# Nat-zewge/cuda-PHDSLAM

Hardware: AMD Instinct MI355X
Metric: PHD update steps/sec at N_particles x N_gm x N_meas; achieved HBM GB/s vs roofline (higher is better)
Workload: dtype f32

## Files before the change

### cuda-phdslam_amd/csrc/phd_kernels.h

```cpp
#pragma once
#include <hip/hip_runtime.h>

#include <cstddef>
#include <cstdint>

#include "phd_device.h"
#include "phd_types.h"

#define PHD_ZBINS 256
#define PHD_STAMP_SLOTS 52
#define UPD_THREADS_MIN 256
#define UPD_THREADS_MAX 1024
#define PHD_CPHD_MAX_M 127
#if defined(PHD_EXPERIMENT) && PHD_EXPERIMENT == 4
#define PHD_CPHD_SEG 2
#elif defined(PHD_EXPERIMENT) && PHD_EXPERIMENT == 5
#define PHD_CPHD_SEG 1
#else
#define PHD_CPHD_SEG 4
#endif

#define PHD_ST_SURVIVOR_OVERFLOW 1
#define PHD_ST_CANDIDATE_OVERFLOW 2
#define PHD_ST_MAP_OVERFLOW 4
#define PHD_ST_SERIAL_MERGE 8
#define PHD_ST_ETA_RANGE 16
#define PHD_ST_PAIR_OVERFLOW 32
#define PHD_ST_WAIT_TIMEOUT 64
#define PHD_ST_INFO (PHD_ST_SERIAL_MERGE | PHD_ST_PAIR_OVERFLOW)

#include <string>

namespace phd {

struct PredictCfg {
    int index_offset;
    float dt;
    int subdivide;
    float l, h, a, b;
    float stdAlpha, stdEncoder;
    float ax, ay, ayaw;
};

struct RsStepArgs {
    const float* w;
    float* w_out;
    int N, B, has_meas;
    float resample_thresh, new_logw;
    uint64_t seed, step;
    double* part_s2;
    unsigned long long *cdf_rel, *part_tot, *part_key;
    unsigned* sync;
    float* out;
    int* parents;
    const phd_pose* pose;
    const int* src;
    phd_pose* new_pose;
    int* new_src;
    float* logw;
    int* err;
};

#define RS_LEAD_WGS 8

struct UpdateArgs {
    int n, cap, M, Mcap, Kcap, Scap;
    int Epool;
    int plreq;
    int Bbuckets;
    int merge_mode;
    const int* slots;
    int first;
    int prio;
    int order;
    unsigned char* hand;
    const int* src;
    int* src_reset;
    const float* map_x;
    const int* size_x;
    const float* map_in;
    float* map_out;
    const int* size_in;
    int* size_out;
    phd_pose* poses;
    float* logw;
    float* logw_out;
    float* delta;
    const float* zr;
    const float* zb;
    const int* zok;
    const float4* zs;
    const unsigned short* zbin;
    int Mv;
    int zwide;
    int* status;
    int* err;
    unsigned long long* stamps;
    int predict;
    phd_ackerman_control pu;
    PredictCfg pc;
    uint64_t pseed, pstep;
    const phd_pose* pose_prior;
    const float* logw_prior;
    float* births;
    int Mb;
    const float* bzr;
    const float* bzb;
    const int* bzvi;
    double* cn_coef;
    int cn_stride;
    const double* lfact;
    int Nmax;
    DevCfg c;
    int rs_lead;
    RsStepArgs rs;
};

__host__ __device__ inline int upd_particle(const UpdateArgs& a, int b, int grid) {
    if (a.slots) return a.slots[b];
    const int g8 = grid & ~7;
    if (a.order == 1 && b < g8) b = g8 - 8 - (b & ~7) + (b & 7);
    return a.first + b;
}

struct UpdLds {
    size_t zr, zb, zok, leta, zs, etafx, etalo, zbin, out, cnt, scr, red, redf, pose, uni, thr;
    size_t u;
    size_t detv;
    size_t mpar, moff, mcur, medge, mpool;
    size_t in, near, skey, skey2;
    size_t skeyidx, gstart;
    size_t total;
    int B;
};

__host__ __device__ inline size_t upd_align16(size_t x) { return (x + 15) & ~(size_t)15; }

#ifndef PHD_RS_OVERLAP
#define PHD_RS_OVERLAP 3
#endif
#ifndef PHD_RS_LEAD
#define PHD_RS_LEAD 1
#endif


#ifndef PHD_PARTC_BMAX
#define PHD_PARTC_BMAX 1024
#endif
static_assert(PHD_PARTC_BMAX == 1024 || PHD_PARTC_BMAX == 2048 || PHD_PARTC_BMAX == 4096,
              "PHD_PARTC_BMAX: 1024, 2048 or 4096 buckets");

__host__ __device__ inline int upd_buckets(int Kcap, int part = 0) {
    return Kcap <= 768 && part == 2 ? 512 : Kcap <= 1024 ? 1024 : Kcap <= 2048 ? 2048 : Kcap <= 8192 ? 4096 : 16384;
}

__host__ __device__ inline int upd_epool(int Kcap) { return (3 * Kcap) / 2 + 16; }

__host__ __device__ inline UpdLds upd_lds_layout(int cap, int Mcap, int Kcap, int Scap, int Epool, int NT,
                                                  int cphd = 0, int part = 0) {
    UpdLds L;
    const int B = upd_buckets(Kcap, part);
    size_t o = 0;
    const bool pz = part != 0;
    L.zr = o;
    o = upd_align16(o + (pz ? 0 : 4 * (size_t)Mcap));
    L.zb = o;
    o = upd_align16(o + (pz ? 0 : 4 * (size_t)Mcap));
    L.zok = o;
    o = upd_align16(o + (pz ? 0 : 4 * (size_t)Mcap));
    L.leta = o;
    o = upd_align16(o + (pz && !(part == 2 && !cphd) ? 0 : 4 * (size_t)Mcap));
    const bool pc = part == 2;
    const bool pa = part == 1;
    L.zs = o;
    o = upd_align16(o + (pc ? 0 : 16 * (size_t)Mcap));
    L.etafx = o;
    o = upd_align16(o + (pc ? 0 : 8 * (size_t)Mcap));
    L.etalo = o;
    o = upd_align16(o + (pc ? 0 : 8 * (size_t)Mcap));
    L.zbin = o;
    o = upd_align16(o + (pc ? 0 : 2 * (size_t)PHD_ZBINS));
    L.out = o;
    o = upd_align16(o + (pc || pa ? 0 : 2 * (size_t)cap));
    L.cnt = o;
    o = upd_align16(o + 4 * 16);
    L.scr = o;
    o = upd_align16(o + (pc ? 4 * 2 * (size_t)(NT / 64) : 4 * 64));
    L.red = o;
    o = upd_align16(o + (pc ? 8 * 4 * (size_t)(NT / 64) : 8 * 64));
    L.redf = o;
    o = upd_align16(o + (pc ? 4 * (32 + (size_t)(NT / 64)) : 4 * 64));
    L.pose = o;
    o = upd_align16(o + sizeof(phd_pose));
    L.uni = o;
    o = upd_align16(o + 8 * 8);
    L.thr = o;
    o = upd_align16(o + (cphd && !pz ? 4 * (size_t)Mcap : 0));
    const size_t c0 = o;
    L.u = o;
    size_t m = c0 + 16 * (size_t)Kcap;
    L.detv = m;
    m = upd_align16(m + (pc ? 0 : 16 * ((size_t)Scap + (cphd ? 0 : (size_t)Mcap))));
    L.mcur = m;
    m = upd_align16(m + 2 * ((size_t)Kcap + 2));
    L.medge = m;
    m = upd_align16(m + 4 * (size_t)Epool);
    L.mpar = m;
    m = upd_align16(m + 2 * (size_t)Kcap);
    L.moff = L.mcur;
    L.mpool = m;
    m = upd_align16(m + 4 * (size_t)Epool);
    size_t table = c0 + (size_t)cap * (8 * 4) + 16 + 2 * (size_t)NT;
    o = upd_align16(part == 1 || (part != 2 && table > m) ? table : m);
    const size_t d0 = o;
    L.in = o;
    o = upd_align16(o + (pc || pa ? 0 : 2 * (size_t)cap));
    L.near = o;
    o = upd_align16(o + (pc || pa ? 0 : 2 * (size_t)cap));
    const size_t skb = upd_align16(4 * ((size_t)Scap + 4));
    if (pc && L.mpool + 4 * (size_t)Epool >= L.mcur + 2 * skb) {
        L.skey = L.mcur;
        L.skey2 = L.mcur + skb;
    } else {
        L.skey = o;
        o = upd_align16(o + (pa ? 0 : skb));
        L.skey2 = o;
        o = upd_align16(o + (pa ? 0 : skb));
    }
    const size_t d_a = o;
    o = d0;
    L.skeyidx = o;
    o = upd_align16(o + 2 * (size_t)Kcap);
    L.B = B;
    int Bp = 0;
    if (part == 2) {
        const int bmin = B > 1024 ? B : 1024;
        for (int b = PHD_PARTC_BMAX > bmin ? PHD_PARTC_BMAX : bmin; b >= bmin && !Bp; b >>= 1)
            if (L.mpar - L.mcur >= 2 * ((size_t)b + 2)) Bp = b;
    }
    if (Bp) {
        L.B = Bp;
        L.gstart = L.mcur;
    } else {
        L.gstart = o;
        o = upd_align16(o + 2 * ((size_t)L.B + 2));
    }
    L.total = (part == 1 || o <= d_a) ? d_a : o;
    return L;
}

struct CphdHand {
    size_t cnt, sums, ehi, elo, in, near, out, skey, leta, thr, misc, detv, table, rb, stride;
};
#define HAND_GIN 0
#define HAND_GNEAR 1
#define HAND_GOUT 2
#define HAND_NSURV 3
#define HAND_FLAGS 4
__host__ __device__ inline CphdHand cphd_hand_layout(int cap, int Mcap, int Scap) {
    CphdHand H;
    size_t o = 0;
    H.cnt = o;
    o += 64;
    H.sums = o;
    o += 32;
    H.ehi = o;
    o = upd_align16(o + 8 * (size_t)Mcap);
    H.elo = o;
    o = upd_align16(o + 8 * (size_t)Mcap);
    H.in = o;
    o = upd_align16(o + 2 * (size_t)cap);
    H.near = o;
    o = upd_align16(o + 2 * (size_t)cap);
    H.out = o;
    o = upd_align16(o + 2 * (size_t)cap);
    H.skey = o;
    o = upd_align16(o + 4 * (size_t)Scap);
    H.leta = o;
    o = upd_align16(o + 4 * (size_t)Mcap);
    H.thr = o;
    o = upd_align16(o + 4 * (size_t)Mcap);
    H.misc = o;
    o = upd_align16(o + 16);
    H.detv = o;
    o = upd_align16(o + 16 * ((size_t)Scap + (size_t)Mcap));
    H.table = o;
    o = upd_align16(o + 32 * (size_t)cap + 16 + 2 * 1024);
    H.rb = o;
    o = upd_align16(o + 8 * (size_t)cap);
    H.stride = (o + 255) & ~(size_t)255;
    return H;
}

__global__ void k_predict_ackerman(phd_pose* poses, int n, phd_ackerman_control u, const phd_ackerman_noise* noise_in,
                                   PredictCfg c, uint64_t seed, uint64_t step, const phd_pose* pose_prior,
                                   const float* logw_prior, float* logw, const int* slots);
__global__ void k_expand(int n, int npp, const phd_pose* pose, const int* src, const float* logw, phd_pose* new_pose,
                         int* new_src, float* new_logw, float log_npp);
__global__ void k_predict_cv(phd_pose* poses, int n, const phd_cv_noise* noise_in, PredictCfg c, uint64_t seed,
                             uint64_t step, const phd_pose* pose_prior, const float* logw_prior, float* logw,
                             const int* slots);
__global__ void k_update_fused_256(UpdateArgs a);
__global__ void k_update_fused_512(UpdateArgs a);
__global__ void k_update_fused_1024(UpdateArgs a);
__global__ void k_update_cphd_a_256(UpdateArgs a);
__global__ void k_update_cphd_a_512(UpdateArgs a);
__global__ void k_update_cphd_a_1024(UpdateArgs a);
__global__ void k_update_cphd_a_p256(UpdateArgs a);
__global__ void k_update_cphd_a_p512(UpdateArgs a);
__global__ void k_update_cphd_c_256(UpdateArgs a);
__global__ void k_update_cphd_c_512(UpdateArgs a);
__global__ void k_update_cphd_c_1024(UpdateArgs a);
__global__ void k_update_phd_a_256(UpdateArgs a);
__global__ void k_update_phd_a_512(UpdateArgs a);
__global__ void k_update_phd_a_1024(UpdateArgs a);
__global__ void k_update_phd_c_256(UpdateArgs a);
__global__ void k_update_phd_c_512(UpdateArgs a);
__global__ void k_update_phd_c_1024(UpdateArgs a);
__global__ void k_cphd_terms(UpdateArgs a);
inline size_t cphd_terms_lds(int Mcap) { return (size_t)7 * 8 * ((size_t)Mcap + 4); }
__global__ void k_cphd_cardinality(const int* src, const double* cn_coef, const double* cn_x, int stride,
                                   const double* lfact, int Nmax, int n, float* out);
__global__ void k_update_fused_p256(UpdateArgs a);
__global__ void k_update_fused_p512(UpdateArgs a);
__global__ void k_update_fused_256_h(UpdateArgs a);
__global__ void k_update_fused_512_h(UpdateArgs a);
__global__ void k_update_fused_1024_h(UpdateArgs a);
__global__ void k_update_fused_p256_h(UpdateArgs a);
__global__ void k_update_fused_p512_h(UpdateArgs a);
__global__ void k_update_phd_c_256_h(UpdateArgs a);
__global__ void k_update_phd_c_512_h(UpdateArgs a);
__global__ void k_update_phd_c_1024_h(UpdateArgs a);
__global__ void k_update_cphd_c_256_h(UpdateArgs a);
__global__ void k_update_cphd_c_512_h(UpdateArgs a);
__global__ void k_update_cphd_c_1024_h(UpdateArgs a);
__global__ void k_normalize(float* logw, int n, const float* lse_override, float* out, float resample_thresh,
                            int has_meas);
__global__ void k_lse_parts(const float* logw, int n, float* out);
__global__ void k_resample(const int* flag, const float* logw_in, float* logw_out, int n, int n_out,
                           const double* u_in,
                           uint64_t seed, uint64_t step, unsigned long long* cdf, int* idx, phd_pose* pose, int* src,
                           phd_pose* tmp_pose, int* tmp_src, float new_logw);
#define RS_LDS_MAX 8192
__global__ void k_normalize_resample(float* logw, int n, float* out, float resample_thresh, int has_meas, uint64_t seed,
                                     uint64_t step, unsigned long long* cdf, int* idx, phd_pose* pose, int* src,
                                     phd_pose* tmp_pose, int* tmp_src, float new_logw);
__global__ void k_apply_parents(const int* flag, const int* idx, int n, phd_pose* pose, int* src, float* logw,
                                phd_pose* tmp_pose, int* tmp_src, float new_logw);
__global__ void k_add_births(int* src, const int* slots, int n, int cap, const float* map_in, const int* size_in,
                             const float* map_x, const int* size_x, float* map_out, int* size_out,
                             const phd_pose* pose, const float* zr, const float* zb, const int* zok, int M, DevCfg c,
                             int* status, int* err);
#define RS_THREADS 1024
#define RS_STAGE_CHUNKS 4
#define RS_MAX_CHUNKS 1024
__global__ void k_rs_max(const float* w, int N, float* part_max);
__global__ void k_rs_sum(const float* w, int N, const float* part_max, int B, double* part_sum, int max_of_w);
__global__ void k_rs_cdf(float* w, int N, const float* part_max, const double* part_sum, int B, double* part_s2,
                         unsigned long long* cdf_rel, unsigned long long* part_tot, unsigned long long* part_key,
                         float* out);
__global__ void k_rs_search(int N, int B, const double* part_s2, const unsigned long long* part_tot,
                            const unsigned long long* part_key, const unsigned long long* cdf_rel,
                            float resample_thresh, int has_meas, uint64_t seed, uint64_t step, int* parents,
                            float* out, const phd_pose* pose, const int* src, phd_pose* new_pose, int* new_src,
                            float* logw, float new_logw, const float* w_norm, unsigned* beyond);
__global__ void k_rs_sumcdf(const float* w, float* w_out, int N, int B, double* part_s2, unsigned long long* cdf_rel,
                            unsigned long long* part_tot, unsigned long long* part_key, float* out);
#define MIG_SENT 0
#define MIG_LSE 1
#define MIG_NEFF 2
#define MIG_FLAG 3
#define MIG_PENDING 4
#define MIG_OVF_SEND 5
#define MIG_OVF_RECV 6
#define MIG_OVF_CAP 7
#define MIG_TIMEOUT 8
#define MIG_SEQ 9
#define MIG_TAIL 10
#define PLAN_ARRIVE0 0
#define PLAN_ARRIVE1 1
// ... 63 lines not shown
```

### cuda-phdslam_amd/csrc/phd_kernels.hip

```cpp
#include <hip/hip_runtime.h>

#include <climits>
#include <cstdint>

#include "phd_detmath.h"
#include "phd_device.h"
#include "phd_kernels.h"
#include "phd_rng.h"
#include "phd_devutil.h"
#include "phd_cphd_terms.h"
#include "phd_block.h"
#include "phd_slab.h"

#ifdef PHD_STAMPS
#define STAMP(k)                                                                                  \
    do {                                                                                          \
        if (threadIdx.x == 0 && a.stamps) a.stamps[(size_t)blockIdx.x * PHD_STAMP_SLOTS + (k)] = __builtin_amdgcn_s_memtime(); \
    } while (0)
#else
#define STAMP(k) \
    do {         \
    } while (0)
#endif
#ifdef PHD_PLAN_STAMPS
// ... 1016 lines not shown
            {
                const int j0 = next_member(-1);
                if (j0 == i && next_member(i) == INT_MAX) {
                    emit_single(dst, cap, slot, X.K.P[i], X.K.V(i));
                    continue;
                }
            }
            for (int j = next_member(-1); j != INT_MAX; j = next_member(j)) {
                const float4 pj = X.K.P[j];
                W += (double)pj.z;
                sx += (double)(pj.z * pj.x);
                sy += (double)(pj.z * pj.y);
            }
            Wf = (float)W;
            const float rW = 1.0f / Wf;
            gx = (float)sx * rW;
            gy = (float)sy * rW;
            for (int j = next_member(-1); j != INT_MAX; j = next_member(j)) {
                const float4 pj = X.K.P[j], vj = X.K.V(j);
                const float d0 = gx - pj.x, d1 = gy - pj.y, w = pj.z;
                cv[0] += (double)(w * (vj.x + d0 * d0));
                cv[1] += (double)(w * (vj.y + d0 * d1));
                cv[2] += (double)(w * (vj.z + d1 * d0));
                cv[3] += (double)(w * (vj.w + d1 * d1));
            }
        }
        emit_merged(dst, cap, slot, Wf, gx, gy, cv);
    }
    return nout;
}

template <bool PRED>
__device__ __forceinline__ phd_pose fused_predict(const UpdateArgs& a, int n) {
    phd_pose ps = a.pose_prior ? a.pose_prior[n] : a.poses[n];
    if (a.logw_prior) a.logw[n] = a.logw_prior[n];
    if (PRED && a.predict) {
        for (int k = 0; k < a.pc.subdivide; k++) {
            const uint64_t st = a.pstep * (uint64_t)a.pc.subdivide + (uint64_t)k;
            if (a.predict == 1) {
                float n_alpha, n_enc;
                ackerman_noise(a.pseed, a.pc.index_offset + n, st, a.pc, &n_alpha, &n_enc);
                ps = predict_ackerman_one(ps, a.pu, n_alpha, n_enc, a.pc);
            } else {
                ps = predict_cv_one(ps, cv_noise(a.pseed, a.pc.index_offset + n, st, a.pc), a.pc);
            }
        }
        a.poses[n] = ps;
    }
    return ps;
}

__global__ void __launch_bounds__(256)
    k_cphd_cardinality(const int* __restrict__ src, const double* __restrict__ cn_coef,
                       const double* __restrict__ cn_x, int stride, const double* __restrict__ lfact, int Nmax,
                       int n, float* __restrict__ out) {
    const int p = blockIdx.x;
    if (p >= n) return;
    const double* co = slab_cn(src ? src[p] : p, cn_coef, cn_x, stride);
    const double ip0 = co[0], lq = co[1], lw = co[2], logW = co[3], W = co[4];
    const int M = (int)co[5];
    for (int k = threadIdx.x; k <= Nmax; k += blockDim.x) {
        double mx = -INFINITY;
        if (k > 0 && !(W > 0)) {
            out[(size_t)p * (Nmax + 1) + k] = PHD_LOG0;
            continue;
        }
        for (int j = 0; j <= min(k, M); j++) {
            const double b = co[6 + j];
            if (b == -INFINITY) continue;
            const double t = b + (k > 0 ? (double)k * logW : 0.0) - W - lfact[k - j] +
                             (k - j > 0 ? (double)(k - j) * lq : 0.0) - (k > 0 ? (double)k * lw : 0.0);
            mx = fmax(mx, t);
        }
        double sum = 0.0;
        if (mx != -INFINITY)
            for (int j = 0; j <= min(k, M); j++) {
                const double b = co[6 + j];
                if (b == -INFINITY) continue;
                const double t = b + (k > 0 ? (double)k * logW : 0.0) - W - lfact[k - j] +
                                 (k - j > 0 ? (double)(k - j) * lq : 0.0) - (k > 0 ? (double)k * lw : 0.0);
                sum += exp(t - mx);
            }
        out[(size_t)p * (Nmax + 1) + k] = mx == -INFINITY ? PHD_LOG0 : (float)(log(sum) + mx - ip0);
    }
}

__device__ __forceinline__ unsigned int bearing_window(float C2, float S0, float S12, float S3, float bearing,
                                                       float floor2, int Mv, const unsigned short* s_zbin) {
    const float k2 = 0.72134752044448170f;
    unsigned int win = (unsigned int)Mv << 16;
    if (!(C2 > floor2) && C2 == C2) return 0;
    const float kap = S3 - S12 * S12 * __builtin_amdgcn_rcpf(4.f * S0);
    if (S0 > 0.f && kap > 0.f && kap < INFINITY && C2 < 1e30f) {
        const float hw = sqrtf(2.f * (C2 - floor2) * __builtin_amdgcn_rcpf(k2 * kap)) * 1.001f + 1e-4f;
        const float ibinw = PHD_ZBINS / 6.28318530717958648f;
        const int ba = (int)floorf((bearing - hw + 3.14159265358979f) * ibinw) - 1;
        const int bc = (int)floorf((bearing + hw + 3.14159265358979f) * ibinw) + 2;
        if (bc - ba < PHD_ZBINS) {
            const int fa = ba >= 0 ? ba / PHD_ZBINS : -((PHD_ZBINS - 1 - ba) / PHD_ZBINS);
            const int fc = bc >= 0 ? bc / PHD_ZBINS : -((PHD_ZBINS - 1 - bc) / PHD_ZBINS);
            const int ia = s_zbin[ba - fa * PHD_ZBINS] + fa * Mv;
            const int ic = s_zbin[bc - fc * PHD_ZBINS] + fc * Mv;
            const int lo = ia - fa * Mv;
            win = (unsigned int)lo | ((unsigned int)min(ic - ia, Mv) << 16);
        }
    }
    return win;
}

__device__ __forceinline__ void eta_term(unsigned long long* ehi, unsigned long long* elo, int m, float q,
                                         float lo_scale, int& flags) {
    flags |= q >= 1048576.f ? PHD_ST_ETA_RANGE : 0;
    const bool hi = q >= 7.62939453125e-06f;
    const unsigned long long y = (unsigned long long)(fminf(q, 4194304.f) * (hi ? 1099511627776.f : lo_scale));
#if PHD_XK == 11
    if (y) (hi ? ehi : elo)[m] += y;
#else
    if (y) atomicAdd((hi ? ehi : elo) + m, y);
#endif
}

template <int NT>
__device__ void rs_step_block(const RsStepArgs& a, unsigned char* smem);

template <int NT, bool PRED, bool CPHD = false, int PART = 0, int METRIC = 0>
__device__ __forceinline__ void update_body(const UpdateArgs& a) {
    static_assert(!CPHD || PART != 0, "the CPHD update runs as three launches (part A, k_cphd_terms, part C)");
    extern __shared__ __attribute__((aligned(16))) unsigned char smem[];
    const int lead = PART == 2 ? a.rs_lead : 0;
    if (PART == 2 && (int)blockIdx.x < lead) {
        if (blockIdx.x == 0) rs_step_block<NT>(a.rs, smem);
        return;
    }
    const int b_ = (int)blockIdx.x - lead, grid_ = (int)gridDim.x - lead;
    const UpdLds L = upd_lds_layout(a.cap, a.Mcap, a.Kcap, a.Scap, a.Epool, NT, CPHD ? 1 : 0, PART);
    float* s_zr = (float*)(smem + L.zr);
    float* s_zb = (float*)(smem + L.zb);
    int* s_zok = (int*)(smem + L.zok);
    float* s_leta = (float*)(smem + L.leta);
    float* s_thr = (float*)(smem + L.thr);
    const float4* s_zs = PART == 2 ? a.zs : (const float4*)(smem + L.zs);
    unsigned long long* s_etafx = (unsigned long long*)(smem + L.etafx);
    unsigned long long* s_etalo = (unsigned long long*)(smem + L.etalo);
    const unsigned short* s_zbin = PART == 2 ? a.zbin : (const unsigned short*)(smem + L.zbin);
    unsigned short* s_out = (unsigned short*)(smem + L.out);
    int* s_cnt = (int*)(smem + L.cnt);
    int* s_scr = (int*)(smem + L.scr);
    double* s_red = (double*)(smem + L.red);
    float* s_redf = (float*)(smem + L.redf);
    unsigned short* s_in = (unsigned short*)(smem + L.in);
    unsigned short* s_near = (unsigned short*)(smem + L.near);
    unsigned int* s_skey = (unsigned int*)(smem + L.skey);
    unsigned int* s_skey2 = (unsigned int*)(smem + L.skey2);
    float4* t_a = (float4*)(smem + L.u);
    float2* t_b = (float2*)(smem + L.u + 16 * (size_t)a.cap);
    unsigned int* t_w = (unsigned int*)(smem + L.u + 24 * (size_t)a.cap);
    int* t_pre = (int*)(smem + L.u + 28 * (size_t)a.cap);
    unsigned short* t_start = (unsigned short*)(smem + L.u + 32 * (size_t)a.cap + 16);
    MergeScratch X;
    X.K.P = (float4*)(smem + L.u);
    X.K.detv = (float4*)(smem + L.detv);
    X.K.cap = a.cap;
    X.par = (short*)(smem + L.mpar);
    X.off = (unsigned short*)(smem + L.moff);
    X.cur = (unsigned short*)(smem + L.mcur);
    X.edges = (unsigned int*)(smem + L.medge);
    X.pool = (unsigned short*)(smem + L.mpool);
    X.plist = (unsigned int*)(smem + L.mpar);
    X.plcap = (int)((L.mpool + 4 * (size_t)a.Epool - L.mpar) / 4);
    X.key = (unsigned short*)(smem + L.skeyidx);
    X.gstart = (unsigned short*)(smem + L.gstart);
    X.st_tests = nullptr;

    const int n = upd_particle(a, b_, grid_);
    const int tid = threadIdx.x;
#ifdef PHD_STAMPS
    if (tid == 0 && a.stamps) a.stamps[(size_t)blockIdx.x * PHD_STAMP_SLOTS + 48] = __builtin_amdgcn_s_memrealtime();
#endif
    const DevCfg& c = a.c;
    const int M = a.M;
    const int sref = a.src ? a.src[n] : n;
    const bool in_x = (sref & PHD_SLAB_X) != 0;
    const int slab = sref & PHD_SLAB_MASK;
    const int G = in_x ? a.size_x[slab] : a.size_in[slab];
    const G1 float* __restrict__ src = g1(uni_p((in_x ? a.map_x : a.map_in) + (size_t)slab * PHD_NF * a.cap));
    const int Mb = a.births ? max(0, min(a.Mb, a.cap - G)) : 0;
    const int Gp = G + Mb;
    G1 float* __restrict__ bdst = a.births ? g1(uni_p(a.births + (size_t)n * PHD_NF * a.cap)) : nullptr;
    const G1 float* __restrict__ bsrc = a.births ? bdst - G : src;
    auto prior = [&](int k) -> const G1 float* { return (k < G ? src : bsrc) + k; };
    X.K.src = src;
    X.K.bsrc = bsrc;
    X.K.G = G;
    G1 float* __restrict__ dst = g1(uni_p(a.map_out + (size_t)n * PHD_NF * a.cap));
    phd_pose& s_pose = *(phd_pose*)(smem + L.pose);
    double* s_uni = (double*)(smem + L.uni);
    if (b_ >= grid_ - a.prio) __builtin_amdgcn_s_setprio(3);
    const CphdHand H = cphd_hand_layout(a.cap, a.Mcap, a.Scap);
    unsigned char* hand = PART ? a.hand + (size_t)n * H.stride : nullptr;
    if (PART == 1) {
        s_out = (unsigned short*)(hand + H.out);
        s_in = (unsigned short*)(hand + H.in);
        s_near = (unsigned short*)(hand + H.near);
        s_skey = (unsigned int*)(hand + H.skey);
    }
    if (PART == 2) {
        s_out = (unsigned short*)(hand + H.out);
        s_in = (unsigned short*)(hand + H.in);
        s_near = (unsigned short*)(hand + H.near);
        X.K.detv = (float4*)(hand + H.detv);
        s_zr = const_cast<float*>(a.zr);
        s_zb = const_cast<float*>(a.zb);
        s_zok = const_cast<int*>(a.zok);
        if (CPHD) {
            s_leta = (float*)(hand + H.leta);
            s_thr = (float*)(hand + H.thr);
        }
        unsigned char* tb = hand + H.table;
        t_a = (float4*)tb;
        t_b = (float2*)(tb + 16 * (size_t)a.cap);
        t_w = (unsigned int*)(tb + 24 * (size_t)a.cap);
        t_pre = (int*)(tb + 28 * (size_t)a.cap);
        t_start = (unsigned short*)(tb + 32 * (size_t)a.cap + 16);
    }
    constexpr int PF = 2;
    float pf[PF][PHD_NF];
#pragma unroll
    for (int it = 0; it < PF; it++) {
        const int k = it * NT + tid;
#pragma unroll
        for (int f = 0; f < PHD_NF; f++) pf[it][f] = (k < G) ? src[f * a.cap + k] : 0.f;
    }
    int hp_cnt[5] = {0, 0, 0, 0, 0};
    unsigned int hp_skey = 0;
    float hp_leta = 0.f, hp_thr = 0.f, hp_nd = 0.f;
    int hp_wide = 0;
    unsigned long long hp_eta[2] = {0ull, 0ull};
    if constexpr (PART == 2) {
        const int* hc = (const int*)(hand + H.cnt);
#pragma unroll
        for (int i = 0; i < 5; i++) hp_cnt[i] = hc[i];
        if (tid < a.Scap) hp_skey = ((const unsigned int*)(hand + H.skey))[tid];
        if (CPHD) {
            if (tid < M) {
                hp_leta = ((const float*)(hand + H.leta))[tid];
                hp_thr = ((const float*)(hand + H.thr))[tid];
            }
            hp_nd = ((const float*)(hand + H.misc))[0];
            hp_wide = ((const int*)(hand + H.misc))[1];
        } else if (tid < M) {
            hp_eta[0] = ((const unsigned long long*)(hand + H.ehi))[tid];
            hp_eta[1] = ((const unsigned long long*)(hand + H.elo))[tid];
        }
    }
    if (tid == 0) s_pose = fused_predict<PRED && PART != 2>(a, n);

    const int Mv = a.Mv;
    for (int m = tid; m < M; m += NT) {
        if (PART == 0) {
            s_zr[m] = a.zr[m];
            s_zb[m] = a.zb[m];
            s_zok[m] = a.zok[m];
        }
        if (PART != 2) {
            s_etafx[m] = 0ull;
            s_etalo[m] = 0ull;
        }
    }
    if (PART != 2) {
        for (int m = tid; m < Mv; m += NT) ((float4*)(smem + L.zs))[m] = a.zs[m];
        for (int b = tid; b < PHD_ZBINS; b += NT) ((unsigned short*)(smem + L.zbin))[b] = a.zbin[b];
    }
    if (tid < 16) s_cnt[tid] = 0;
    __syncthreads();
    const phd_pose pose = s_pose;
    STAMP(0);

    const float k2 = 0.72134752044448170f;
    double card_d = 0.0;
    double win_d = 0.0, qd_d = 0.0, wall_d = 0.0;
    int n1r = 0, n2r = 0, n0r = 0;
    constexpr int NW = NT / 64;
    const float lpd = d_safe_log(c.pd);
    for (int base = 0; base < (PART == 2 ? 0 : Gp); base += NT) {
        const int k = base + tid;
        int cls = -1;
        float4 ta = make_float4(0.f, 0.f, 0.f, 0.f);
        float2 tb = make_float2(0.f, 0.f);
        unsigned int win = 0;
        if (k < Gp) {
            float v[PHD_NF];
            if (k >= G) {
                const int m = a.bzvi[k - G];
                float mean[2], cov[4];
                d_birth(c, pose.px, pose.py, pose.ptheta, a.bzr[m], a.bzb[m], mean, cov);
                v[0] = c.birthWeight;
                v[1] = mean[0];
                v[2] = mean[1];
                v[3] = cov[0];
                v[4] = cov[1];
                v[5] = cov[2];
                v[6] = cov[3];
#pragma unroll
                for (int f = 0; f < PHD_NF; f++) bdst[f * a.cap + (k - G)] = v[f];
            } else if (base == 0) {
#pragma unroll
                for (int f = 0; f < PHD_NF; f++) v[f] = pf[0][f];
            } else if (base == NT) {
#pragma unroll
                for (int f = 0; f < PHD_NF; f++) v[f] = pf[1][f];
            } else {
#pragma unroll
                for (int f = 0; f < PHD_NF; f++) v[f] = src[f * a.cap + k];
            }
            const float dx = v[1] - pose.px;
            const float dy = v[2] - pose.py;
            const float r2 = dx * dx + dy * dy;
            const float r = sqrtf(r2);
            const float bearing = d_wrap((PHD_XK == 13 ? atan2f(dy, dx) : phd_atan2f(dy, dx)) - pose.ptheta);
            const float ab = fabsf(bearing);
            if (CPHD) wall_d += (double)v[0];
            if (r >= c.minRange && r <= c.maxRange && ab <= c.maxBearing)
                cls = 1;
            else if ((double)r >= 0.8 * (double)c.minRange && (double)r <= 1.2 * (double)c.maxRange &&
                     (double)ab <= 1.2 * (double)c.maxBearing)
                cls = 2;
            else
                cls = 0;
            if (cls == 1) {
                const float w = v[0];
                DevEkf e;
                d_ekf_from_geometry(c, dx, dy, r2, r, bearing, v[3], v[4], v[5], v[6], e);
                const double lc =
                    (double)((e.pd > 0.f ? lpd : PHD_LOG0) + d_safe_log(w)) - c.log_2pi - 0.5 * (double)d_safe_log(e.det);
                const float C2 = (float)(1.4426950408889634 * lc);
                const float S12 = e.S1 + e.S2;
                ta = make_float4(e.r, e.bearing, e.S0, S12);
                tb = make_float2(e.S3, C2);
                card_d += (double)(e.pd * w);
                if (CPHD) {
                    win_d += (double)w;
                    qd_d += (double)(1 - e.pd) * (double)w;
                }
                win = bearing_window(C2, e.S0, S12, e.S3, e.bearing, c.walk_floor, Mv, s_zbin);
            }
        }
        const int lane = tid & 63, wid = tid >> 6;
        const unsigned long long b1 = __ballot(cls == 1), b2 = __ballot(cls == 2), b0 = __ballot(cls == 0);
        const unsigned long long lt = (1ull << lane) - 1ull;
        int* sb = s_scr + 16 + ((base / NT) & 1) * 3 * NW;
        if (lane == 0) {
            sb[wid] = __popcll(b1);
            sb[NW + wid] = __popcll(b2);
            sb[2 * NW + wid] = __popcll(b0);
        }
        __syncthreads();
        int o1 = n1r, o2 = n2r, o0 = n0r, t1 = 0, t2 = 0, t0 = 0;
#pragma unroll
        for (int w = 0; w < NW; w++) {
            const int c1 = sb[w], c2 = sb[NW + w], c0 = sb[2 * NW + w];
            if (w < wid) {
                o1 += c1;
                o2 += c2;
                o0 += c0;
            }
            t1 += c1;
            t2 += c2;
            t0 += c0;
        }
        if (cls == 1) {
            const int j = o1 + __popcll(b1 & lt);
            s_in[j] = (unsigned short)k;
            t_a[j] = ta;
            t_b[j] = tb;
            t_w[j] = win;
            if (PART == 1) {
                G1 float* rbp = (G1 float*)(hand + H.rb) + 2 * j;
                rbp[0] = ta.x;
                rbp[1] = ta.y;
            }
        }
        if (cls == 2) s_near[o2 + __popcll(b2 & lt)] = (unsigned short)k;
        if (cls == 0) s_out[o0 + __popcll(b0 & lt)] = (unsigned short)k;
        n1r += t1;
        n2r += t2;
        n0r += t0;
    }
    if (PART != 2 && tid == 0) {
        s_cnt[0] = n1r;
        s_cnt[1] = n2r;
        s_cnt[2] = n0r;
    }
    int Gin = PART == 2 ? s_cnt[0] : n1r;
    STAMP(1);
    if constexpr (PART == 2) {
    } else if (CPHD) {
        double v[4] = {card_d, win_d, qd_d, wall_d};
        block_sum<4, NT>(v, s_red);
        if (tid == 0) {
            s_uni[0] = v[0];
            s_uni[1] = v[1];
            s_uni[2] = v[2];
            s_uni[3] = v[3];
        }
    } else {
        double v[1] = {card_d};
        block_sum<1, NT>(v, s_red);
        if (tid == 0) s_uni[0] = v[0];
    }
    STAMP(2);
    {
        const float thr2 = c.lq_keep_thresh * 1.4426950408889634f;
        const float lo_scale = a.cap <= 2047 ? 1.1805916207174113e21f : 1.152921504606846976e18f;
        const int lane = tid & 63;
        const unsigned long long lt = (1ull << lane) - 1ull;
        int eflags = 0;
        int W = 0, chunk = 0;
        auto plan_walk = [&]() {
            W = 0;
            for (int base = 0; base < Gin; base += NT) {
                const int j = base + tid;
                const int units = j < Gin ? (int)((t_w[j] >> 16) + 3) >> 2 : 0;
                int tot;
                const int pre = block_excl_scan<NT>(units, s_scr, &tot);
                if (j < Gin) t_pre[j] = W + pre;
                W += tot;
// ... 8 lines not shown
            __syncthreads();
        };
        auto walk = [&](const int pass) {
        const bool do_sum = pass == 0;
        const float thr_u = CPHD ? c.cphd_thr0 : thr2;
        const int w0 = tid * chunk, w1 = min(w0 + chunk, W);
#ifdef PHD_STAMPS
        int st_pairs = 0, st_qpos = 0;
#endif
        int j = w0 < w1 ? t_start[tid] : 0;
        STAMP(25);
        int jbeg = t_pre[j], jend = t_pre[j + 1];
        for (int it = 0; it < (PHD_XK == 1 ? 0 : chunk); it++) {
            const int w = w0 + it;
            const bool act = w < w1;
            if (act && w == jend) {
                j++;
                while (t_pre[j + 1] <= w) j++;
                jbeg = t_pre[j];
                jend = t_pre[j + 1];
            }
            const float4 ta = t_a[j];
            const float2 tb = t_b[j];
            const unsigned int win = t_w[j];
            const int cnt = act ? (int)(win >> 16) : 0;
            const int e0 = 4 * (w - jbeg);
            int ms = (int)(win & 0xffffu) + (act ? e0 : 0);
            while (ms >= Mv) ms -= Mv;
            float4 z[4];
#pragma unroll
            for (int k = 0; k < 4; k++) {
                z[k] = s_zs[ms];
                ms = (ms + 1 == Mv) ? 0 : ms + 1;
            }
            float l2q[4];
            int mm[4];
#pragma unroll
            for (int k = 0; k < 4; k++) {
                const float i0 = z[k].x - ta.x;
                float i1 = z[k].y - ta.y;
                if (fabsf(i1) > 3.14159250f) i1 = d_wrap(i1);
                const float u = __builtin_fmaf(i0, ta.z, i1 * ta.w);
                const float dist = __builtin_fmaf(i0, u, i1 * i1 * tb.x);
                l2q[k] = e0 + k < cnt ? __builtin_fmaf(-k2, dist, tb.y) : -INFINITY;
                mm[k] = __float_as_int(z[k].z);
            }
            if (do_sum) {
#pragma unroll
                for (int k = 0; k < 4; k++) {
                    const float q = __builtin_amdgcn_exp2f(l2q[k]);
                    if (PHD_XK != 12 && q > 0.f) eta_term(s_etafx, s_etalo, mm[k], q, lo_scale, eflags);
#ifdef PHD_STAMPS
                    st_pairs += e0 + k < cnt;
                    st_qpos += q > 0.f;
#endif
                }
            }
            bool lst[4];
#pragma unroll
            for (int k = 0; k < 4; k++) lst[k] = l2q[k] >= (pass == 0 ? thr_u : s_thr[e0 + k < cnt ? mm[k] : 0]);
            unsigned long long bl[4];
#pragma unroll
            for (int k = 0; k < 4; k++) bl[k] = __ballot(lst[k]);
            const int c0 = __popcll(bl[0]), c1 = __popcll(bl[1]), c2 = __popcll(bl[2]), c3 = __popcll(bl[3]);
            const int ntot = c0 + c1 + c2 + c3;
            if (ntot) {
                int base = 0;
                if (lane == 0) base = atomicAdd(&s_cnt[3], ntot);
                base = __shfl(base, 0, 64);
                const int off[4] = {base, base + c0, base + c0 + c1, base + c0 + c1 + c2};
#pragma unroll
                for (int k = 0; k < 4; k++) {
                    const int sl = off[k] + __popcll(bl[k] & lt);
                    if (lst[k] && sl < a.Scap) s_skey[sl] = ((unsigned int)mm[k] << 16) | (unsigned int)j;
                }
            }
        }
#ifdef PHD_STAMPS
        atomicAdd(&s_cnt[8 + pass], st_pairs);
        atomicAdd(&s_cnt[10 + pass], st_qpos);
#endif
        if (eflags) atomicOr(&s_cnt[14], eflags);
        __syncthreads();
        };
        if constexpr (PART != 2) {
        plan_walk();
#ifdef PHD_STAMPS
        if (tid == 0) s_cnt[12] = W;
#endif
        STAMP(21);
        walk(0);
        if constexpr (PART == 1) {
            int* hc = (int*)(hand + H.cnt);
            if (tid == 0) {
                hc[HAND_GIN] = Gin;
                hc[HAND_GNEAR] = s_cnt[1];
                hc[HAND_GOUT] = s_cnt[2];
                hc[HAND_NSURV] = s_cnt[3];
                hc[HAND_FLAGS] = s_cnt[14];
            }
            if (tid < 4) ((double*)(hand + H.sums))[tid] = s_uni[tid];
            for (int m = tid; m < M; m += NT) {
                ((unsigned long long*)(hand + H.ehi))[m] = s_etafx[m];
                ((unsigned long long*)(hand + H.elo))[m] = s_etalo[m];
            }
            if constexpr (!CPHD) {
                static_assert(NT >= 256, "one measurement per thread (M <= 256)");
                float lt = 0.f;
                if (tid < M) {
                    float sum;
                    if (Gin > 0) {
                        double sd = (double)s_etafx[tid] * 9.094947017729282e-13 +
                                    (double)s_etalo[tid] * (a.cap <= 2047 ? 8.470329472543003e-22 : 8.673617379884035e-19);
                        sd += (double)c.kappa;
                        sd += (double)c.birthWeight;
                        sum = (float)sd;
                    } else {
                        sum = c.kappa + c.birthWeight;
                    }
                    lt = d_det_safe_log(sum);
                }
                __syncthreads();
                if (tid < M) ((float*)s_etafx)[tid] = lt;
                __syncthreads();
                if (tid == 0) {
                    float pw = 0.f;
                    for (int m = 0; m < M; m++) pw += ((const float*)s_etafx)[m];
                    const float cardp = (float)(s_uni[0] + (double)M * (double)c.birthWeight);
                    const float delta = pw - cardp;
                    a.delta[n] = delta;
                    const float nw = a.logw[n] + delta;
                    a.logw[n] = nw;
                    if (a.logw_out) a.logw_out[n] = nw;
                }
            }
            STAMP(9);
            return;
        }
        } else {
            if (tid == 0) {
                s_cnt[0] = hp_cnt[HAND_GIN];
                s_cnt[1] = hp_cnt[HAND_GNEAR];
                s_cnt[2] = hp_cnt[HAND_GOUT];
                s_cnt[3] = hp_cnt[HAND_NSURV];
                s_cnt[14] = hp_cnt[HAND_FLAGS];
                ((float*)(s_uni + 4))[0] = hp_nd;
                ((float*)(s_uni + 4))[1] = phd_det_expf(hp_nd);
                s_uni[5] = (double)hp_wide;
                if (!CPHD) s_uni[0] = ((const double*)(hand + H.sums))[0];
            }
            Gin = hp_cnt[HAND_GIN];
            const int nsk = min(hp_cnt[HAND_NSURV], a.Scap);
            for (int q = tid; q < nsk; q += NT) s_skey[q] = q == tid ? hp_skey : ((const unsigned int*)(hand + H.skey))[q];
            __syncthreads();
            if (CPHD && (s_uni[5] != 0.0 || s_cnt[3] > a.Scap)) {
                float tm = INFINITY;
                for (int m = tid; m < M; m += NT) tm = fminf(tm, s_thr[m]);
                const float fl = fminf(c.walk_floor, -block_max_f<NT>(-tm, s_redf) - 1.f);
                for (int q = tid; q < Gin; q += NT) {
                    const int k = s_in[q];
                    const G1 float* sk = prior(k);
                    const float dx = sk[1 * a.cap] - pose.px;
                    const float dy = sk[2 * a.cap] - pose.py;
                    const float r2 = dx * dx + dy * dy;
                    const float r = sqrtf(r2);
                    const float bearing = d_wrap(phd_atan2f(dy, dx) - pose.ptheta);
                    DevEkf e;
                    d_ekf_from_geometry(c, dx, dy, r2, r, bearing, sk[3 * a.cap], sk[4 * a.cap], sk[5 * a.cap],
                                        sk[6 * a.cap], e);
                    const double lc = (double)(d_safe_log(e.pd) + d_safe_log(sk[0])) - c.log_2pi -
                                      0.5 * (double)d_safe_log(e.det);
                    const float C2 = (float)(1.4426950408889634 * lc);
                    const float S12 = e.S1 + e.S2;
                    t_a[q] = make_float4(e.r, e.bearing, e.S0, S12);
                    t_b[q] = make_float2(e.S3, C2);
                    t_w[q] = bearing_window(C2, e.S0, S12, e.S3, e.bearing, fl, Mv, s_zbin);
                }
                __syncthreads();
                plan_walk();
                if (tid == 0) s_cnt[3] = 0;
                __syncthreads();
                walk(1);
            }
        }
        STAMP(22);
        if (!CPHD && tid < M) {
            float sum;
            if (Gin > 0) {
                const unsigned long long ehi = PART == 2 ? hp_eta[0] : s_etafx[tid];
                const unsigned long long elo = PART == 2 ? hp_eta[1] : s_etalo[tid];
                double sd = (double)ehi * 9.094947017729282e-13 +
                            (double)elo * (a.cap <= 2047 ? 8.470329472543003e-22 : 8.673617379884035e-19);
                sd += (double)c.kappa;
                sd += (double)c.birthWeight;
                sum = (float)sd;
            } else {
                sum = c.kappa + c.birthWeight;
            }
            s_leta[tid] = d_det_safe_log(sum);
        }
        __syncthreads();
    }
    if (!CPHD && PART != 2 && tid == 0) {
        float pw = 0.f;
        for (int m = 0; m < M; m++) pw += s_leta[m];
        const float cardp = (float)(s_uni[0] + (double)M * (double)c.birthWeight);
        const float delta = pw - cardp;
        a.delta[n] = delta;
        const float nw = a.logw[n] + delta;
        a.logw[n] = nw;
        if (a.logw_out) a.logw_out[n] = nw;
    }
    STAMP(3);
    int nsurv = s_cnt[3];
    int flags = s_cnt[14];
    if (Mb < (a.births ? a.Mb : 0)) flags |= PHD_ST_MAP_OVERFLOW;
    if (nsurv > a.Scap) {
        flags |= PHD_ST_SURVIVOR_OVERFLOW;
        nsurv = a.Scap;
    }

    {
        int* b_cnt = (int*)(smem + L.u);
        int* b_base = b_cnt + 264;
        unsigned short* b_pos = (unsigned short*)(b_base + 264);
        unsigned int* b_tmp = (unsigned int*)(smem + L.u + 2 * 264 * 4 + upd_align16(2 * (size_t)a.Scap));
        for (int m = tid; m <= M; m += NT) b_cnt[m] = 0;
        __syncthreads();
        for (int s = tid; s < nsurv; s += NT)
            b_pos[s] = (unsigned short)atomicAdd(&b_cnt[s_skey[s] >> 16], 1);
        __syncthreads();
        {
            int run = 0;
            for (int base = 0; base < M; base += NT) {
                const int m = base + tid;
                int tot;
                const int pre = block_excl_scan<NT>(m < M ? b_cnt[m] : 0, s_scr, &tot);
                if (m < M) b_base[m] = run + pre;
                run += tot;
            }
        }
        __syncthreads();
        for (int s = tid; s < nsurv; s += NT) {
            const unsigned int key = s_skey[s];
            b_tmp[b_base[key >> 16] + b_pos[s]] = key;
        }
        __syncthreads();
        for (int s = tid; s < nsurv; s += NT) {
            const unsigned int key = s_skey[s];
            const int m = (int)(key >> 16), b0 = b_base[m], nb = b_cnt[m];
            int r = 0;
            for (int q = 0; q < nb; q++) r += b_tmp[b0 + q] < key;
            s_skey2[b0 + r] = key;
        }
        __syncthreads();
    }

    STAMP(4);
    int ncand = 0;
    int sbc = 0;
    int sc_bad = 0;
    float sc_lmax = 0.f;
    for (int base = 0; base < (PHD_XK == 4 ? 0 : Gin); base += NT) {
        const int j = base + tid;
        float w = 0.f;
        bool keep = false;
        int k = 0;
        float v[PHD_NF];
        if (j < Gin) {
            k = s_in[j];
            if (PART == 2 && base == 0 && k == j && k < G) {
#pragma unroll
                for (int f = 0; f < PHD_NF; f++) v[f] = pf[0][f];
            } else if (PART == 2 && base == NT && k == j && k < G) {
#pragma unroll
                for (int f = 0; f < PHD_NF; f++) v[f] = pf[1][f];
            } else {
#pragma unroll
                for (int f = 0; f < PHD_NF; f++) v[f] = prior(k)[f * a.cap];
            }
            w = CPHD ? (v[0] > 0.f ? v[0] * ((const float*)(s_uni + 4))[1] : 0.f) : v[0] * (1 - c.pd);
            keep = !(w < c.minFeatureWeight);
        }
        int tot;
        const int r = block_rank<NT, false>(keep, sb_at<NT>(s_scr, sbc), &tot);
        if (keep) {
            const int p = ncand + r;
            if (p < a.Kcap) {
                const float4 vc = make_float4(v[3], v[4], v[5], v[6]);
                X.K.P[p] = cand_record<METRIC>(v[1], v[2], w, vc, c.minSeparation, sc_bad, sc_lmax, (unsigned)k);
            }
        }
        ncand += tot;
    }
    STAMP(5);
    const int nd0 = min(ncand, a.Kcap);
    for (int base = 0; base < (PHD_XK == 4 ? 0 : nsurv); base += NT) {
        const int s = base + tid;
        bool keep = false;
        float w = 0.f, mx = 0.f, my = 0.f;
        DevEkf e;
        if (s < nsurv) {
            const unsigned int key = s_skey2[s];
            const int m = (int)(key >> 16);
            const int j = (int)(key & 0xffffu);
            const int k = s_in[j];
            const G1 float* sk = prior(k);
            mx = sk[1 * a.cap];
            my = sk[2 * a.cap];
            if constexpr (PART == 2) {
                const G1 float* rbp = (const G1 float*)(hand + H.rb) + 2 * j;
                const float dx = mx - s_pose.px, dy = my - s_pose.py;
                d_ekf_from_geometry(c, dx, dy, dx * dx + dy * dy, rbp[0], rbp[1], sk[3 * a.cap], sk[4 * a.cap],
                                    sk[5 * a.cap], sk[6 * a.cap], e);
            } else {
                d_compute_ekf(c, s_pose.px, s_pose.py, s_pose.ptheta, mx, my, sk[3 * a.cap], sk[4 * a.cap],
                              sk[5 * a.cap], sk[6 * a.cap], e);
            }
            const float i0 = s_zr[m] - e.r;
            const float i1 = d_wrap(s_zb[m] - e.bearing);
            const float dist = i0 * i0 * e.S0 + i0 * i1 * (e.S1 + e.S2) + i1 * i1 * e.S3;
            const float g = (float)(-0.5 * (double)dist - c.log_2pi - 0.5 * (double)d_safe_log(e.det));
            const float lq = d_safe_log(e.pd) + d_safe_log(sk[0]) + g;
            w = expf(lq - s_leta[m]);
            keep = !(w < c.minFeatureWeight);
            mx = mx + e.K0 * i0 + e.K2 * i1;
            my = my + e.K1 * i0 + e.K3 * i1;
        }
        int tot;
        const int r = block_rank<NT, false>(keep, sb_at<NT>(s_scr, sbc), &tot);
        if (keep) {
            const int p = ncand + r;
            if (p < a.Kcap) {
                const float4 v = make_float4(e.cu0, e.cu1, e.cu2, e.cu3);
                X.K.P[p] = cand_record<METRIC>(mx, my, w, v, c.minSeparation, sc_bad, sc_lmax,
                                               0x8000u | (unsigned)(p - nd0));
                X.K.detv[p - nd0] = v;
            }
        }
        ncand += tot;
    }
    STAMP(6);
    for (int base = 0; base < (CPHD ? 0 : M); base += NT) {
        const int m = base + tid;
        bool keep = false;
        float w = 0.f;
        if (m < M) {
            const float lb = s_zok[m] ? c.log_birth : PHD_LOG0;
            w = expf(lb - s_leta[m]);
            keep = !(w < c.minFeatureWeight);
        }
        int tot;
        const int r = block_rank<NT, false>(keep, sb_at<NT>(s_scr, sbc), &tot);
        if (keep) {
            const int p = ncand + r;
            if (p < a.Kcap) {
                float mean[2], cov[4];
                d_birth(c, s_pose.px, s_pose.py, s_pose.ptheta, s_zr[m], s_zb[m], mean, cov);
                const float4 v = make_float4(cov[0], cov[1], cov[2], cov[3]);
                X.K.P[p] = cand_record<METRIC>(mean[0], mean[1], w, v, c.minSeparation, sc_bad, sc_lmax,
                                               0x8000u | (unsigned)(p - nd0));
                X.K.detv[p - nd0] = v;
            }
        }
        ncand += tot;
    }
    const int Gnear = s_cnt[1];
    for (int q = tid; q < Gnear; q += NT) {
        const int p = ncand + q;
        if (p < a.Kcap) {
            const int k = s_near[q];
            const G1 float* sk = prior(k);
            const float4 v = make_float4(sk[3 * a.cap], sk[4 * a.cap], sk[5 * a.cap], sk[6 * a.cap]);
            X.K.P[p] = cand_record<METRIC>(sk[1 * a.cap], sk[2 * a.cap], sk[0], v, c.minSeparation, sc_bad, sc_lmax,
                                           (unsigned)k);
        }
    }
    ncand += Gnear;
    if (ncand > a.Kcap) {
        flags |= PHD_ST_CANDIDATE_OVERFLOW;
        ncand = a.Kcap;
    }
    __syncthreads();

    STAMP(7);
    int nout = (PHD_XK == 3 || PHD_XK == 4) ? 0
               : a.merge_mode != 0         ? -1
                                           : merge_parallel<NT, METRIC>(X, ncand, c.minSeparation, dst, a.cap, a.Epool,
                                                                        a.Bbuckets, s_scr, s_redf, s_cnt + 3, sc_bad,
                                                                        sc_lmax, a);
    if (nout < 0) {
        __syncthreads();
        nout = merge_serial<NT, METRIC>(X.K, nullptr, ncand, X.par, c.minSeparation, dst, a.cap, s_red, s_redf);
        flags |= PHD_ST_SERIAL_MERGE;
    }

    STAMP(8);
    flags |= s_cnt[14] & PHD_ST_PAIR_OVERFLOW;
    const int Gout = s_cnt[2];
    for (int q = tid; q < Gout; q += NT) {
        const int p = nout + q;
        if (p < a.cap) {
            const int k = s_out[q];
#pragma unroll
            for (int f = 0; f < PHD_NF; f++) st_out(dst + f * a.cap + p, prior(k)[f * a.cap]);
        }
    }
    int total = nout + Gout;
    if (total > a.cap) {
        flags |= PHD_ST_MAP_OVERFLOW;
        total = a.cap;
    }
    if (tid == 0) {
        a.size_out[n] = total;
        a.status[n] = flags;
        if (flags & ~PHD_ST_INFO) {
            atomicOr(a.err, flags & ~PHD_ST_INFO);
            atomicAdd(a.err + 3, 1);
        }
        if (flags & PHD_ST_SERIAL_MERGE) atomicAdd(a.err + 1, 1);
        if (a.src_reset) a.src_reset[n] = n;
    }
    STAMP(9);
#ifdef PHD_STAMPS
    if (tid == 0 && a.stamps) a.stamps[(size_t)blockIdx.x * PHD_STAMP_SLOTS + 49] = __builtin_amdgcn_s_memrealtime();
    if (tid == 0 && a.stamps) a.stamps[(size_t)blockIdx.x * PHD_STAMP_SLOTS + 10] = ((unsigned long long)ncand << 32) | (unsigned)nsurv;
    if (tid == 0 && a.stamps) {
        a.stamps[(size_t)blockIdx.x * PHD_STAMP_SLOTS + 40] = ((unsigned long long)s_cnt[8] << 32) | (unsigned)s_cnt[10];
        a.stamps[(size_t)blockIdx.x * PHD_STAMP_SLOTS + 41] = ((unsigned long long)s_cnt[9] << 32) | (unsigned)s_cnt[11];
        a.stamps[(size_t)blockIdx.x * PHD_STAMP_SLOTS + 42] = ((unsigned long long)Gin << 32) | (unsigned)s_cnt[12];
    }
#endif
}

typedef const __attribute__((address_space(4))) UpdateArgs KArgs;
__device__ __forceinline__ const UpdateArgs& kargs(const UpdateArgs& a) {
    (void)a;
    unsigned long long v = (unsigned long long)__builtin_amdgcn_kernarg_segment_ptr();
    asm volatile("" : "+s"(v));
    return *(const UpdateArgs*)(KArgs*)v;
}

__global__ void __launch_bounds__(256) k_update_fused_256(UpdateArgs a) { update_body<256, false>(kargs(a)); }
__global__ void __launch_bounds__(512) __attribute__((amdgpu_waves_per_eu(6, 8))) k_update_fused_512(UpdateArgs a) {
    update_body<512, false>(kargs(a));
}
__global__ void __launch_bounds__(1024) k_update_fused_1024(UpdateArgs a) { update_body<1024, false>(kargs(a)); }
__global__ void __launch_bounds__(256) k_update_fused_p256(UpdateArgs a) { update_body<256, true>(kargs(a)); }
#define PHD_CPHD_WPE __attribute__((amdgpu_waves_per_eu(4, 8)))
__global__ void __launch_bounds__(512) k_update_fused_p512(UpdateArgs a) { update_body<512, true>(kargs(a)); }
__global__ void __launch_bounds__(256) __attribute__((amdgpu_waves_per_eu(6, 8))) k_update_cphd_a_256(UpdateArgs a) {
    update_body<256, false, true, 1>(kargs(a));
}
__global__ void __launch_bounds__(512) k_update_cphd_a_512(UpdateArgs a) { update_body<512, false, true, 1>(kargs(a)); }
__global__ void __launch_bounds__(1024) k_update_cphd_a_1024(UpdateArgs a) { update_body<1024, false, true, 1>(kargs(a)); }
__global__ void __launch_bounds__(256) __attribute__((amdgpu_waves_per_eu(6, 8))) k_update_cphd_a_p256(UpdateArgs a) {
    update_body<256, true, true, 1>(kargs(a));
}
__global__ void __launch_bounds__(512) k_update_cphd_a_p512(UpdateArgs a) { update_body<512, true, true, 1>(kargs(a)); }
// ... 1518 lines not shown
```

Baseline: 3721.

## Prefetch more prior features and cache survivor indices in PART 2 update

In the PART==2 path, the prior prefetch grows to three register tiles read through prior(k) up to Gp, so more candidates take their features from registers instead of a fresh global load. A new shared array s_skk stores each survivor's prior index next to the sorted keys, removing a dependent s_in lookup in the survivor loop. Zeroing of the bucket counts moves to the kernel prologue, where it shares an existing barrier, and the bucket scan alternates scratch slots so it can skip a barrier. The cost is more registers, a little extra LDS for s_skk, and extra index bookkeeping.

```diff
diff --git a/cuda-phdslam_amd/csrc/phd_kernels.h b/cuda-phdslam_amd/csrc/phd_kernels.h
--- a/cuda-phdslam_amd/csrc/phd_kernels.h
+++ b/cuda-phdslam_amd/csrc/phd_kernels.h
@@ -129,6 +129,7 @@
     size_t detv;
     size_t mpar, moff, mcur, medge, mpool;
     size_t in, near, skey, skey2;
+    size_t skk;
     size_t skeyidx, gstart;
     size_t total;
     int B;
@@ -218,14 +219,18 @@
     L.near = o;
     o = upd_align16(o + (pc || pa ? 0 : 2 * (size_t)cap));
     const size_t skb = upd_align16(4 * ((size_t)Scap + 4));
-    if (pc && L.mpool + 4 * (size_t)Epool >= L.mcur + 2 * skb) {
+    const size_t skq = pc ? upd_align16(2 * ((size_t)Scap + 4)) : 0;
+    if (pc && L.mpool + 4 * (size_t)Epool >= L.mcur + 2 * skb + skq) {
         L.skey = L.mcur;
         L.skey2 = L.mcur + skb;
+        L.skk = L.mcur + 2 * skb;
     } else {
         L.skey = o;
         o = upd_align16(o + (pa ? 0 : skb));
         L.skey2 = o;
         o = upd_align16(o + (pa ? 0 : skb));
+        L.skk = o;
+        o = upd_align16(o + skq);
     }
     const size_t d_a = o;
     o = d0;
diff --git a/cuda-phdslam_amd/csrc/phd_kernels.hip b/cuda-phdslam_amd/csrc/phd_kernels.hip
--- a/cuda-phdslam_amd/csrc/phd_kernels.hip
+++ b/cuda-phdslam_amd/csrc/phd_kernels.hip
@@ -1192,6 +1192,7 @@
     unsigned short* s_near = (unsigned short*)(smem + L.near);
     unsigned int* s_skey = (unsigned int*)(smem + L.skey);
     unsigned int* s_skey2 = (unsigned int*)(smem + L.skey2);
+    unsigned short* s_skk = (unsigned short*)(smem + L.skk);
     float4* t_a = (float4*)(smem + L.u);
     float2* t_b = (float2*)(smem + L.u + 16 * (size_t)a.cap);
     unsigned int* t_w = (unsigned int*)(smem + L.u + 24 * (size_t)a.cap);
@@ -1263,16 +1264,22 @@
         t_pre = (int*)(tb + 28 * (size_t)a.cap);
         t_start = (unsigned short*)(tb + 32 * (size_t)a.cap + 16);
     }
-    constexpr int PF = 2;
+    constexpr int PF = PART == 2 ? 3 : 2;
     float pf[PF][PHD_NF];
 #pragma unroll
     for (int it = 0; it < PF; it++) {
         const int k = it * NT + tid;
-#pragma unroll
-        for (int f = 0; f < PHD_NF; f++) pf[it][f] = (k < G) ? src[f * a.cap + k] : 0.f;
+        if constexpr (PART == 2) {
+#pragma unroll
+            for (int f = 0; f < PHD_NF; f++) pf[it][f] = (k < Gp) ? prior(k)[f * a.cap] : 0.f;
+        } else {
+#pragma unroll
+            for (int f = 0; f < PHD_NF; f++) pf[it][f] = (k < G) ? src[f * a.cap + k] : 0.f;
+        }
     }
     int hp_cnt[5] = {0, 0, 0, 0, 0};
     unsigned int hp_skey = 0;
+    int hq_k = 0;
     float hp_leta = 0.f, hp_thr = 0.f, hp_nd = 0.f;
     int hp_wide = 0;
     unsigned long long hp_eta[2] = {0ull, 0ull};
@@ -1312,6 +1319,9 @@
         for (int b = tid; b < PHD_ZBINS; b += NT) ((unsigned short*)(smem + L.zbin))[b] = a.zbin[b];
     }
     if (tid < 16) s_cnt[tid] = 0;
+    if constexpr (PART == 2) {
+        for (int m = tid; m <= M; m += NT) ((int*)(smem + L.u))[m] = 0;
+    }
     __syncthreads();
     const phd_pose pose = s_pose;
     STAMP(0);
@@ -1626,6 +1636,7 @@
             Gin = hp_cnt[HAND_GIN];
             const int nsk = min(hp_cnt[HAND_NSURV], a.Scap);
             for (int q = tid; q < nsk; q += NT) s_skey[q] = q == tid ? hp_skey : ((const unsigned int*)(hand + H.skey))[q];
+            if (tid < nsk) hq_k = s_in[hp_skey & 0xffffu];
             __syncthreads();
             if (CPHD && (s_uni[5] != 0.0 || s_cnt[3] > a.Scap)) {
                 float tm = INFINITY;
@@ -1655,6 +1666,7 @@
                 if (tid == 0) s_cnt[3] = 0;
                 __syncthreads();
                 walk(1);
+                if (tid < min(s_cnt[3], a.Scap)) hq_k = s_in[s_skey[tid] & 0xffffu];
             }
         }
         STAMP(22);
@@ -1699,8 +1711,10 @@
         int* b_base = b_cnt + 264;
         unsigned short* b_pos = (unsigned short*)(b_base + 264);
         unsigned int* b_tmp = (unsigned int*)(smem + L.u + 2 * 264 * 4 + upd_align16(2 * (size_t)a.Scap));
-        for (int m = tid; m <= M; m += NT) b_cnt[m] = 0;
-        __syncthreads();
+        if constexpr (PART != 2) {
+            for (int m = tid; m <= M; m += NT) b_cnt[m] = 0;
+            __syncthreads();
+        }
         for (int s = tid; s < nsurv; s += NT)
             b_pos[s] = (unsigned short)atomicAdd(&b_cnt[s_skey[s] >> 16], 1);
         __syncthreads();
@@ -1709,7 +1723,7 @@
             for (int base = 0; base < M; base += NT) {
                 const int m = base + tid;
                 int tot;
-                const int pre = block_excl_scan<NT>(m < M ? b_cnt[m] : 0, s_scr, &tot);
+                const int pre = block_excl_scan<NT, false>(m < M ? b_cnt[m] : 0, s_scr + ((base / NT) & 1) * (NT / 64), &tot);
                 if (m < M) b_base[m] = run + pre;
                 run += tot;
             }
@@ -1726,6 +1740,7 @@
             int r = 0;
             for (int q = 0; q < nb; q++) r += b_tmp[b0 + q] < key;
             s_skey2[b0 + r] = key;
+            if constexpr (PART == 2) s_skk[b0 + r] = (unsigned short)(s == tid ? hq_k : (int)s_in[key & 0xffffu]);
         }
         __syncthreads();
     }
@@ -1742,14 +1757,19 @@
         int k = 0;
         float v[PHD_NF];
         if (j < Gin) {
-            k = s_in[j];
-            if (PART == 2 && base == 0 && k == j && k < G) {
-#pragma unroll
-                for (int f = 0; f < PHD_NF; f++) v[f] = pf[0][f];
-            } else if (PART == 2 && base == NT && k == j && k < G) {
-#pragma unroll
-                for (int f = 0; f < PHD_NF; f++) v[f] = pf[1][f];
-            } else {
+            bool have = false;
+            k = (PART == 2 && Gin == Gp) ? j : (int)s_in[j];
+            if constexpr (PART == 2) {
+#pragma unroll
+                for (int it = 0; it < PF; it++) {
+                    if (base == it * NT && k == j) {
+                        have = true;
+#pragma unroll
+                        for (int f = 0; f < PHD_NF; f++) v[f] = pf[it][f];
+                    }
+                }
+            }
+            if (!have) {
 #pragma unroll
                 for (int f = 0; f < PHD_NF; f++) v[f] = prior(k)[f * a.cap];
             }
@@ -1778,7 +1798,7 @@
             const unsigned int key = s_skey2[s];
             const int m = (int)(key >> 16);
             const int j = (int)(key & 0xffffu);
-            const int k = s_in[j];
+            const int k = PART == 2 ? (int)s_skk[s] : (int)s_in[j];
             const G1 float* sk = prior(k);
             mx = sk[1 * a.cap];
             my = sk[2 * a.cap];
```

New measurement: 3732, median of 6. Within noise of the previous version (+0.3%).
